# robustrobotics/multi_view_stereonet

Measured on AMD Instinct MI355X. Metric: depthmaps/sec at 512x256, 64 hypotheses, 2 src views; L1 vs ref, higher is better.
Workload: dtype f32; 1 GPU; GTA-SfM-shaped 512x256, D=64 hypotheses, 2 source views, cost-volume filter + 5 refiners; global_batch=256, parallelism=dp1 (independent images, all-gather of metric rows)

## Files before the change

### multi_view_stereonet_amd/csrc/mvsn_conv_wino.hip

```cpp
#include <type_traits>
#include <utility>

#include "mvsn_resident.h"
#include "mvsn_conv_wino.h"

namespace mvsn {

constexpr int WN_THREADS = 512, WN_WAVES = 8;
constexpr int WN_TY = 16, WN_TX = 32;
constexpr int WN_WIDE_TY = 10, WN_WIDE_TX = 40, WN_WIDE_PC = WN_WIDE_TX / 2, WN_WIDE_NP = (WN_WIDE_TY / 2) * WN_WIDE_PC;
constexpr int WN_ROLL_PR = 6, WN_ROLL_NP = WN_ROLL_PR * WN_WIDE_PC, WN_ROLL_HY = 2 * WN_ROLL_PR + 3;
constexpr int WN_TILE_RP = 3;
constexpr int wn_pa(int dil) { return (dil + 3) / 4 * 4; }
constexpr int WN_UFLOATS = 16 * 128;
constexpr int WN_MAX_CHUNKS = 9;
constexpr int WN_LDS_MAX = 160 * 1024;

__device__ floatx4 g_wn_zero16 = {0.f, 0.f, 0.f, 0.f};

#ifndef MVSN_WN_ABLATE
#define MVSN_WN_ABLATE 0
#endif

#ifndef MVSN_RD_ABLATE
// ... 796 lines not shown
#pragma unroll
      for (int rr = 0; rr < 2; ++rr) {
        const bool rok = rr ? row1 : row0;
#pragma unroll
        for (int h = 0; h < 2; ++h) {
          const bool ok = rok && (h ? q1 : q0);
          if (rok && (!(MVSN_WN_ABLATE & 64) || n < 0))
            wn_store4<MVSN_WN_NT_STORES ? 2 : 0>(
                osrd, h ? ovoff1 : ovoff0, (unsigned)(((size_t)(t * 16) * cstride + (size_t)rr * DIL * g.W) * 4),
                floatx4{y[t][rr][4 * h], y[t][rr][4 * h + 1], y[t][rr][4 * h + 2], y[t][rr][4 * h + 3]});
          if (ok) {
#pragma unroll
            for (int k = 0; k < 4; ++k) s[t] += y[t][rr][4 * h + k];
          }
        }
      }
    }
    WN_STAMP();
    if (out_partials != nullptr) {
      auto sum8 = [](float v) {
        v += dpp_mov<0xB1>(v);
        v += dpp_mov<0x4E>(v);
        v += dpp_mov<0x141>(v);
        return v;
      };
      const int hi = (lq >> 3) & 1;
      const float npos = 8.0f * (float)cnt;
      const float rn = cnt == 16 ? 0.0078125f : (cnt == 8 ? 0.015625f : (cnt == 4 ? 0.03125f : 0.0f));
      float m[2], qv[2] = {0.f, 0.f};
#pragma unroll
      for (int t = 0; t < 2; ++t) {
        s[t] = sum8(s[t]);
        m[t] = s[t] * rn;
      }
#pragma unroll
      for (int t = 0; t < 2; ++t)
#pragma unroll
        for (int rr = 0; rr < 2; ++rr)
#pragma unroll
          for (int h = 0; h < 2; ++h)
            if ((rr ? row1 : row0) && (h ? q1 : q0)) {
#pragma unroll
              for (int k = 0; k < 4; ++k) {
                const float dv = y[t][rr][4 * h + k] - m[t];
                qv[t] += dv * dv;
              }
            }
#pragma unroll
      for (int t = 0; t < 2; ++t) qv[t] = sum8(qv[t]);
      int rtile = tile_id, rwave = wave;
      bool rec_ok = true;
      if constexpr (RP) {
        const int yq = oy & (TY - 1);
        rtile = (oy / TY) * g.ntx + x0 / TX, rwave = yq / (2 * DIL) * DIL + yq % DIL;
        rec_ok = oy < g.nty * TY;
      }
      if ((lq & 7) == 0 && rec_ok) {
        float *rec = out_partials + (((size_t)n * (RP ? g.tiles : ptiles) + (size_t)z * g.tiles + rtile) * WN_WAVES + rwave) * 48;
        rec += gq * 12 + hi * 3;
#pragma unroll
        for (int t = 0; t < 2; ++t) {
          rec[t * 6 + 0] = npos;
          rec[t * 6 + 1] = m[t];
          rec[t * 6 + 2] = qv[t];
        }
      }
    }
  };

  auto finish_tile_tr = [&](int n, int z, int tile_id, int y0, int x0, int r_s) {
    int lq;
    asm volatile("v_mbcnt_lo_u32_b32 %0, -1, 0\n\tv_mbcnt_hi_u32_b32 %0, -1, %0" : "=v"(lq));
    const int pc = lq & 15, gq = lq >> 4;
    int oy = y0 + 2 * wave, ox = x0 + 2 * pc;
    bool slot_ok = true;
    unsigned zb = 0;
    if constexpr (WIDE != 0) {
      const int q = wave * 16 + pc;
      slot_ok = q < NP;
      const int qq = slot_ok ? q : 0, pr = qq / WN_WIDE_PC;
      oy = y0 + 2 * pr, ox = x0 + 2 * (qq - pr * WN_WIDE_PC);
      if constexpr (ROLL) {
        const bool pb = pr >= r_s;
        oy = pb ? 2 * (pr - r_s) : oy;
        zb = pb ? (unsigned)plane : 0u;
        slot_ok = slot_ok & (!pb | (z + 1 < g.D));
      }
    }
    const bool row0 = oy < g.H, row1 = oy + 1 < g.H, cok = slot_ok && ox < g.W;
    const size_t cstride = VOL ? (size_t)g.D * plane : plane;
    const __amdgpu_buffer_rsrc_t osrd = wn_rsrc(out + (size_t)n * 32 * cstride + (size_t)z * plane, (unsigned)(32 * cstride * 4));
    const unsigned ovoff = cok ? ((unsigned)(4 * gq) * (unsigned)cstride + zb + (unsigned)(oy * g.W + ox)) * 4u : 0xFFFFFFFFu;
    const unsigned ovoff0 = (!WIDE || row0) ? ovoff : 0xFFFFFFFFu, ovoff1 = (!WIDE || row1) ? ovoff : 0xFFFFFFFFu;
    float s[2] = {0.f, 0.f};
    float y[2][4][4];
#pragma unroll
    for (int t = 0; t < 2; ++t) {
      const floatx4 bv = *reinterpret_cast<const floatx4 *>(bias_lds + t * 16 + 4 * gq);
#pragma unroll
      for (int r = 0; r < 4; ++r) {
        float s0[4], s1[4];
#pragma unroll
        for (int j = 0; j < 4; ++j) {
          s0[j] = acc[j][t][r] + acc[4 + j][t][r] + acc[8 + j][t][r];
          s1[j] = acc[4 + j][t][r] - acc[8 + j][t][r] - acc[12 + j][t][r];
        }
        y[t][r][0] = s0[0] + s0[1] + s0[2] + bv[r];
        y[t][r][1] = s0[1] - s0[2] - s0[3] + bv[r];
        y[t][r][2] = s1[0] + s1[1] + s1[2] + bv[r];
        y[t][r][3] = s1[1] - s1[2] - s1[3] + bv[r];
        if (!(MVSN_WN_ABLATE & 64) || n < 0) {
          const unsigned so = (unsigned)((size_t)(t * 16 + r) * cstride * 4);
          if (WIDE || row0) wn_store2<MVSN_WN_NT_TR ? 2 : 0>(osrd, ovoff0, so, y[t][r][0], y[t][r][1]);
          if (WIDE || row1) wn_store2<MVSN_WN_NT_TR ? 2 : 0>(osrd, ovoff1, so + (unsigned)g.W * 4u, y[t][r][2], y[t][r][3]);
        }
        if (row0 && cok) s[t] += y[t][r][0] + y[t][r][1];
        if (row1 && cok) s[t] += y[t][r][2] + y[t][r][3];
      }
    }
    WN_STAMP();
    if (out_partials != nullptr) {
      auto sum16 = [](float v) {
        v += dpp_mov<0xB1>(v);
        v += dpp_mov<0x4E>(v);
        v += dpp_mov<0x141>(v);
        v += dpp_mov<0x140>(v);
        return v;
      };
      const int vp = (g.W - x0) >> 1;
      float npos = (float)(8 * ((row0 ? 1 : 0) + (row1 ? 1 : 0)) * (vp > 16 ? 16 : vp));
      if constexpr (WIDE != 0)
        npos = sum16(cok ? (float)(8 * ((row0 ? 1 : 0) + (row1 ? 1 : 0))) : 0.0f);
      float m[2], qv[2] = {0.f, 0.f};
#pragma unroll
      for (int t = 0; t < 2; ++t) {
        s[t] = sum16(s[t]);
        m[t] = npos > 0.f ? s[t] / npos : 0.f;
      }
#pragma unroll
      for (int t = 0; t < 2; ++t)
#pragma unroll
        for (int r = 0; r < 4; ++r)
#pragma unroll
          for (int k = 0; k < 4; ++k)
            if ((k < 2 ? row0 : row1) && cok) {
              const float dv = y[t][r][k] - m[t];
              qv[t] += dv * dv;
            }
#pragma unroll
      for (int t = 0; t < 2; ++t) qv[t] = sum16(qv[t]);
      if (pc < 4) {
        float *rec = out_partials + (((size_t)n * ptiles + (ROLL ? (size_t)0 : (size_t)z * g.tiles) + tile_id) * WN_WAVES + wave) * 48;
        rec += gq * 12 + pc * 3;
        const int ga = gq >> 1;
        const bool a = pc == ga, b = pc == 2 + ga;
        rec[0] = (a || b) ? npos : 0.f;
        rec[1] = a ? m[0] : (b ? m[1] : 0.f);
        rec[2] = a ? qv[0] : (b ? qv[1] : 0.f);
      }
    }
  };

  int step = 0, mm_stage = 0;
  for (int round = 0; round < my_items; ++round) {
#ifdef MVSN_WN_STAMPS
    dbg_on = round >= 3 || my_items < 4;
#endif
    const int flat = g.rev ? total - 1 - (round * G + slot) : round * G + slot;
    const int n = flat / ptiles;
    int tile_id = flat - n * ptiles, z = 0;
    int r_pr0 = 0, r_s = WN_ROLL_PR;
    if constexpr (ROLL) {
      roll_item(tile_id, z, r_pr0, r_s);
    } else if constexpr (VOL) {
      z = tile_id / g.tiles;
      tile_id -= z * g.tiles;
    }
    const int tyi = ROLL ? 0 : wdiv(tile_id, g.fd_ntx), txi = ROLL ? 0 : tile_id - tyi * g.ntx;
    const int y0 = ROLL ? 2 * r_pr0 : item_y0(tyi), x0 = txi * TX;

#pragma unroll
    for (int xi = 0; xi < 16; ++xi) asm volatile("" : "=v"(acc[xi][0]), "=v"(acc[xi][1]));

    int chunk = 0;
    auto do_step = [&](auto firstc) {
      const bool has_next = step + 1 < total_steps;
      bool waited = false;
      if constexpr (RIDE > 0) {
        if constexpr (ASM_RIDE) {
          if (rd_young != PERV) asm volatile("s_waitcnt vmcnt(0)" ::: "memory");
          asm volatile("s_waitcnt vmcnt(%0)" ::"n"(PERV) : "memory");
        } else if (rd_young == PERV) asm volatile("s_waitcnt vmcnt(%0)" ::"n"(PERV) : "memory");
        else if (rd_young == PER) asm volatile("s_waitcnt vmcnt(%0)" ::"n"(PER) : "memory");
        else if (VOL && rd_young == 2) asm volatile("s_waitcnt vmcnt(2)" ::: "memory");
        else asm volatile("s_waitcnt vmcnt(0)" ::: "memory");
        rd_consume(lane);
        waited = true;
      }
      if (has_next) {
        const int rest = total_steps - (step + 2);
        if (!waited) wait_landed(rest < 0 ? 0 : (rest < NSTAGE - 2 ? rest : NSTAGE - 2));
        xf_apply();
        WN_STAMP();
        if (!(MVSN_WN_ABLATE & 8)) wn_barrier<LDS_BARRIER>();
        if (MVSN_WN_STAGGER > 0 && wave >= 4) __builtin_amdgcn_s_sleep(MVSN_WN_STAGGER);
        WN_STAMP();
        xf_prepare();
      }
      rd_issue(flat, chunk);
      float dn[KS][4][4];
      if (has_next && !(MVSN_WN_ABLATE & 32)) {
        if (MVSN_WN_XF == 1) tr_load(dn);
        else if (MVSN_WN_XF == 0) tr_load(dn, 0, 1);
      }
      auto multiply = [&](auto first, auto hc) {
        constexpr bool FIRST = decltype(first)::value;
        constexpr int h = decltype(hc)::value;
        const float *ub = U + (VOL ? mm_stage : chunk) * UST + h * WN_UFLOATS + lane;
        float fb[2][2];
        fb[0][0] = ub[0], fb[0][1] = ub[64];
        auto tcol = [&](int i, int j) {
          const float d0 = dn[h][0][dslot(j)], d1 = dn[h][1][dslot(j)], d2 = dn[h][2][dslot(j)], d3 = dn[h][3][dslot(j)];
          return i == 0 ? d0 - d2 : (i == 1 ? d1 + d2 : (i == 2 ? d2 - d1 : d1 - d3));
        };
        constexpr bool INTER = MVSN_WN_XF == 1 || (MVSN_WN_XF == 0 && h == 0);
        float tc[4], tn[4];
        if constexpr (INTER) {
#pragma unroll
          for (int j = 0; j < 4; ++j) tc[j] = tcol(0, j);
        } else {
          if (has_next && !(MVSN_WN_ABLATE & 32)) tr_load(dn, h, h + 1);
        }
#pragma unroll
        for (int xi = 0; xi < 16; ++xi) {
          const int cur = xi & 1, ti = xi >> 2, tj = xi & 3;
          if (INTER && ti < 3) tn[tj] = tcol(ti + 1, tj);
          if (xi + 1 < 16 && !(MVSN_WN_ABLATE & 2)) {
            fb[cur ^ 1][0] = ub[(xi + 1) * 128];
            fb[cur ^ 1][1] = ub[(xi + 1) * 128 + 64];
          }
          if constexpr (FIRST) {
            acc[xi][0] = TR ? mfma16x16x4(fb[cur][0], v[h][xi], floatx4{0.f, 0.f, 0.f, 0.f})
                            : mfma16x16x4(v[h][xi], fb[cur][0], floatx4{0.f, 0.f, 0.f, 0.f});
            acc[xi][1] = TR ? mfma16x16x4(fb[cur][1], v[h][xi], floatx4{0.f, 0.f, 0.f, 0.f})
                            : mfma16x16x4(v[h][xi], fb[cur][1], floatx4{0.f, 0.f, 0.f, 0.f});
          } else {
            acc[xi][0] = TR ? mfma16x16x4(fb[cur][0], v[h][xi], acc[xi][0]) : mfma16x16x4(v[h][xi], fb[cur][0], acc[xi][0]);
            acc[xi][1] = TR ? mfma16x16x4(fb[cur][1], v[h][xi], acc[xi][1]) : mfma16x16x4(v[h][xi], fb[cur][1], acc[xi][1]);
          }
          if (h == 0 && xi == 1 && has_next && !(MVSN_WN_ABLATE & 4)) {
            pf_issue();
            uq_issue();
          }
          if constexpr (INTER) {
            if (!(MVSN_WN_ABLATE & 1)) {
              v[h][xi] = tj == 0 ? tc[0] - tc[2] : (tj == 1 ? tc[1] + tc[2] : (tj == 2 ? tc[2] - tc[1] : tc[1] - tc[3]));
              if (MVSN_WN_PIN) asm volatile("" : "+v"(v[h][xi]));
            }
            if (tj == 3) {
#pragma unroll
              for (int k = 0; k < 4; ++k) tc[k] = tn[k];
            }
          }
          __builtin_amdgcn_sched_barrier(0);
        }
        if constexpr (!INTER) {
          if (!(MVSN_WN_ABLATE & 1)) {
            tr_finish(dn, v, h, h + 1);
#pragma unroll
            for (int xi = 0; xi < 16; ++xi)
              if (MVSN_WN_PIN) asm volatile("" : "+v"(v[h][xi]));
          }
          __builtin_amdgcn_sched_barrier(0);
        }
      };
      multiply(firstc, std::integral_constant<int, 0>{});
      if constexpr (KS == 2) multiply(std::false_type{}, std::integral_constant<int, 1>{});
      tr_advance();
      if constexpr (VOL) mm_stage = mm_stage + 1 == NSTAGE ? 0 : mm_stage + 1;
      WN_STAMP();
      ++step;
    };
    do_step(std::true_type{});
    for (chunk = 1; chunk < nsteps; ++chunk) do_step(std::false_type{});
    if (!(MVSN_WN_ABLATE & 16) || n < 0) {
      if constexpr (TR) finish_tile_tr(n, z, tile_id, y0, x0, r_s);
      else finish_tile(n, z, tile_id, y0, x0);
    }
  }
  if constexpr (RIDE > 0) {
    if (total_steps > 0) {
      asm volatile("s_waitcnt vmcnt(0)" ::: "memory");
      int ln;
      asm volatile("v_mbcnt_lo_u32_b32 %0, -1, 0\n\tv_mbcnt_hi_u32_b32 %0, -1, %0" : "=v"(ln));
      rd_consume(ln);
    }
  }
#ifdef MVSN_WN_STAMPS
  if (dbg)
    for (int i = 0; i < dbg_i; ++i) dbg[i] = dbg_lds[i];
#endif
}

constexpr int S2_TY = 16, S2_TX = 32;
constexpr int S2_ROWS = 2 * S2_TY + 3, S2_XS = 2 * S2_TX + 8, S2_DQ = S2_XS / 4;
constexpr int S2_GROUPS = S2_ROWS * S2_DQ, S2_PIECES = (S2_GROUPS + 63) / 64;
constexpr int S2_RCST = S2_ROWS * S2_XS + 1;
constexpr int S2_STAGE = 4 * S2_RCST;
constexpr int S2_UST = 4 * WN_UFLOATS;
constexpr int S2_STEPS = 8;
constexpr size_t S2_LDS_BYTES = (size_t)(2 * S2_STAGE + 2 * S2_UST + 32) * sizeof(float);
static_assert(S2_PIECES * 4 % WN_WAVES == 0, "a step's raw pieces divide evenly among the waves");
static_assert(S2_LDS_BYTES <= 160 * 1024, "LDS plan");

__global__ void wino_s2_pack_kernel(const float *__restrict__ w, float *__restrict__ out) {
  const int idx = blockIdx.x * blockDim.x + threadIdx.x;
  if (idx >= S2_STEPS * S2_UST) return;
  const int lane = idx & 63, t = (idx >> 6) & 1, xi = (idx >> 7) & 15, ph = (idx >> 11) & 3, cc = idx >> 13;
  const int py = ph >> 1, px = ph & 1;
  const int co = t * 16 + (lane & 15), ci = cc * 4 + (lane >> 4);
  const float *g = w + ((size_t)co * 32 + ci) * 25;
  const float G[4][3] = {{1.f, 0.f, 0.f}, {0.5f, 0.5f, 0.5f}, {0.5f, -0.5f, 0.5f}, {0.f, 0.f, 1.f}};
  const int i = xi >> 2, j = xi & 3;
  float u = 0.0f;
  for (int a = 0; a < 3; ++a)
    for (int b = 0; b < 3; ++b) {
      const int ky = 2 * a + py, kx = 2 * b + px;
      if (ky < 5 && kx < 5) u += G[i][a] * g[ky * 5 + kx] * G[j][b];
    }
  out[idx] = u;
}

#ifndef MVSN_S2_PIN
#define MVSN_S2_PIN 1
#endif
#ifndef MVSN_S2_CNTWAIT
#define MVSN_S2_CNTWAIT 1
#endif
struct WinoS2Args {
  int n, H, W, Ho, Wo, ntx, tiles;
  WinoDiv fd_ntx;
};

__global__ __launch_bounds__(WN_THREADS, 2) void conv_wino_s2_kernel(WinoS2Args g, const float *__restrict__ in,
                                                                     const float *__restrict__ upk,
                                                                     const float *__restrict__ bias,
                                                                     float *__restrict__ out) {
  extern __shared__ __attribute__((aligned(16))) float smem[];
  float *U = smem + 2 * S2_STAGE;
  float *bias_lds = U + 2 * S2_UST;
  const int tid = threadIdx.x, lane = tid & 63;
  const int wave = __builtin_amdgcn_readfirstlane(tid >> 6);
  const size_t plane = (size_t)g.H * g.W;
  const int oplane = g.Ho * g.Wo;
  const int total = g.n * g.tiles, G = gridDim.x;
  const int slot = xcd_tile_index(blockIdx.x, G);
  const int my_items = slot < total ? (total - slot + G - 1) / G : 0;
  const int total_steps = my_items * S2_STEPS;
  if (tid < 32) bias_lds[tid] = bias ? bias[tid] : 0.0f;

  constexpr int PER = S2_PIECES * 4 / WN_WAVES;
  const int dch = wave >> 1, dp0 = (wave & 1) * PER;
  int pf_item = 0, pf_cc = 0, pf_n = 0;
  int pf_goff[PER];
  auto pf_plan = [&]() {
    const int flat = pf_item * G + slot;
    const int n = flat / g.tiles, tile = flat - n * g.tiles;
    const int tyi = wdiv(tile, g.fd_ntx), txi = tile - tyi * g.ntx;
    const int gy0 = 2 * tyi * S2_TY - 2, gx0 = 2 * txi * S2_TX - 4;
    pf_n = n;
    int lo;
    asm volatile("v_mbcnt_lo_u32_b32 %0, -1, 0\n\tv_mbcnt_hi_u32_b32 %0, -1, %0" : "=v"(lo));
#pragma unroll
    for (int i = 0; i < PER; ++i) {
      const int e = (dp0 + i) * 64 + lo;
      const int row = e / S2_DQ, q = e - row * S2_DQ;
      const int gy = gy0 + row, gx = gx0 + 4 * q;
      pf_goff[i] = (gy >= 0 && gy < g.H && gx >= 0 && gx < g.W) ? (gy * g.W + gx) * 4 : -1;
    }
  };
  auto pf_issue = [&](int step) {
    if (step >= total_steps) return;
    const float *src = in + ((size_t)pf_n * 32 + pf_cc * 4 + dch) * plane;
    float *dst = smem + (step & 1) * S2_STAGE + dch * S2_RCST;
#pragma unroll
    for (int i = 0; i < PER; ++i)
      if ((dp0 + i) * 64 + lane < S2_GROUPS)
        wn_dma16_buf<true>(src, (unsigned)plane * 4u, (unsigned)pf_goff[i], dst + (dp0 + i) * 256);
    const float *us = upk + (size_t)pf_cc * S2_UST + wave * 1024 + lane * 4;
    float *ud = U + (step & 1) * S2_UST + wave * 1024;
#pragma unroll
    for (int i = 0; i < 4; ++i) wn_dma16<true>(us + i * 256, ud + i * 256);
    if (++pf_cc == S2_STEPS) {
      pf_cc = 0;
      ++pf_item;
      if (pf_item < my_items) pf_plan();
    }
  };
  if (my_items > 0) pf_plan();
  pf_issue(0);

  const int pcol = lane & 15, kc = lane >> 4;
  const int rbase = kc * S2_RCST + (4 * wave) * S2_XS + 4 * pcol + 2;

  floatx4 acc[16][2];
#pragma unroll
  for (int xi = 0; xi < 16; ++xi) acc[xi][0] = acc[xi][1] = floatx4{0.f, 0.f, 0.f, 0.f};

  int item = 0, cc = 0;
  for (int step = 0; step < total_steps; ++step) {
    if (MVSN_S2_CNTWAIT && cc == 0 && step > 0) asm volatile("s_waitcnt vmcnt(8)" ::: "memory");
    else asm volatile("s_waitcnt vmcnt(0)" ::: "memory");
    wn_barrier<true>();
    pf_issue(step + 1);
    const float *raw = smem + (step & 1) * S2_STAGE + rbase;
    const float *us = U + (step & 1) * S2_UST + lane;
#pragma unroll
    for (int py = 0; py < 2; ++py) {
      typedef float s2_f2 __attribute__((ext_vector_type(2)));
      s2_f2 d[4][4];
#pragma unroll
      for (int i = 0; i < 4; ++i)
#pragma unroll
        for (int j = 0; j < 4; ++j) {
          const float *q = raw + (py + 2 * i) * S2_XS + 2 * j;
          d[i][j] = (py && i == 3) ? s2_f2{0.f, 0.f} : s2_f2{q[0], q[1]};
        }
      s2_f2 t[4][4], v[16];
#pragma unroll
      for (int j = 0; j < 4; ++j) {
        t[0][j] = d[0][j] - d[2][j];
        t[1][j] = d[1][j] + d[2][j];
        t[2][j] = d[2][j] - d[1][j];
        t[3][j] = d[1][j] - d[3][j];
      }
#pragma unroll
      for (int i = 0; i < 4; ++i) {
        v[i * 4 + 0] = t[i][0] - t[i][2];
        v[i * 4 + 1] = t[i][1] + t[i][2];
        v[i * 4 + 2] = t[i][2] - t[i][1];
        v[i * 4 + 3] = t[i][1] - t[i][3];
      }
      if (MVSN_S2_PIN) {
#pragma unroll
        for (int xi = 0; xi < 16; ++xi)
          if (!(py && (xi >> 2) == 3)) asm volatile("" : "+v"(v[xi]));
      }
#pragma unroll
      for (int xi = 0; xi < 16; ++xi) {
        if (py && (xi >> 2) == 3) continue;
        const float *u = us + ((py * 2) * 16 + xi) * 128;
        acc[xi][0] = mfma16x16x4(v[xi].x, u[0], acc[xi][0]);
        acc[xi][1] = mfma16x16x4(v[xi].x, u[64], acc[xi][1]);
        if ((xi & 3) != 3) {
          acc[xi][0] = mfma16x16x4(v[xi].y, u[16 * 128], acc[xi][0]);
          acc[xi][1] = mfma16x16x4(v[xi].y, u[16 * 128 + 64], acc[xi][1]);
        }
      }
    }
    if (++cc == S2_STEPS) {
      cc = 0;
      const int flat = item * G + slot;
      const int n = flat / g.tiles, tile = flat - n * g.tiles;
      const int tyi = wdiv(tile, g.fd_ntx), txi = tile - tyi * g.ntx;
      const int y0 = tyi * S2_TY + 2 * wave, x0 = txi * S2_TX;
      const __amdgpu_buffer_rsrc_t osrd = wn_rsrc(out + (size_t)n * 32 * oplane, (unsigned)(32 * oplane) * 4u);
      int lo;
      asm volatile("v_mbcnt_lo_u32_b32 %0, -1, 0\n\tv_mbcnt_hi_u32_b32 %0, -1, %0" : "=v"(lo));
      const int ocl = lo & 15, oq = lo >> 4;
      unsigned ovoff[2];
#pragma unroll
      for (int hx = 0; hx < 2; ++hx)
        ovoff[hx] = x0 + 8 * oq + 4 * hx < g.Wo ? (unsigned)((ocl * oplane + 8 * oq + 4 * hx) * 4) : 0xFFFFFFFFu;
#pragma unroll
      for (int tt = 0; tt < 2; ++tt) {
        const float bv = bias_lds[tt * 16 + ocl];
        float y[4][2][2];
#pragma unroll
        for (int r = 0; r < 4; ++r) {
          float tm[2][4];
#pragma unroll
          for (int j = 0; j < 4; ++j) {
            tm[0][j] = acc[0 + j][tt][r] + acc[4 + j][tt][r] + acc[8 + j][tt][r];
            tm[1][j] = acc[4 + j][tt][r] - acc[8 + j][tt][r] - acc[12 + j][tt][r];
          }
#pragma unroll
          for (int a = 0; a < 2; ++a) {
            y[r][a][0] = tm[a][0] + tm[a][1] + tm[a][2] + bv;
            y[r][a][1] = tm[a][1] - tm[a][2] - tm[a][3] + bv;
          }
        }
#pragma unroll
        for (int a = 0; a < 2; ++a) {
          const bool rok = y0 + a < g.Ho;
          const unsigned so = rok ? (unsigned)((tt * 16 * oplane + (y0 + a) * g.Wo + x0) * 4) : 0u;
          wn_store4<0>(osrd, rok ? ovoff[0] : 0xFFFFFFFFu, so, floatx4{y[0][a][0], y[0][a][1], y[1][a][0], y[1][a][1]});
          wn_store4<0>(osrd, rok ? ovoff[1] : 0xFFFFFFFFu, so, floatx4{y[2][a][0], y[2][a][1], y[3][a][0], y[3][a][1]});
        }
      }
#pragma unroll
      for (int xi = 0; xi < 16; ++xi) acc[xi][0] = acc[xi][1] = floatx4{0.f, 0.f, 0.f, 0.f};
      ++item;
    }
  }
}

static int g_wn_rowphase = 0;

bool wino_geom(const mvsn_conv_desc *d, WinoGeom *g) {
  if (!d || d->precision != MVSN_CONV_FP32_WINO) return false;
  g->rpy = 0;
  if (d->n <= 0 || d->c_in <= 0 || d->c_out != 32 || d->depth < 1 || d->rows <= 0 || d->cols <= 0) return false;
  g->s2 = false;
  if (d->kd == 1 && d->kh == 5 && d->kw == 5 && d->stride == 2) {
    if (d->c_in != 32 || d->dilation != 1 || d->depth != 1 || d->cols % 8 != 0) return false;
    if ((unsigned long long)d->rows * d->cols * 32ull * 4ull >= (1ull << 31)) return false;
    g->s2 = true, g->wide = 0;
    g->n = d->n, g->cin = 32, g->H = d->rows, g->W = d->cols, g->dil = 1, g->D = 1, g->vol = false;
    g->nty = ((d->rows - 1) / 2 + 1 + S2_TY - 1) / S2_TY;
    g->ntx = ((d->cols - 1) / 2 + 1 + S2_TX - 1) / S2_TX;
    g->tiles = g->nty * g->ntx;
    g->nchunks = S2_STEPS * 4;
    g->packed_floats = (size_t)S2_STEPS * S2_UST;
    return (long)g->n * g->tiles < (1L << 30);
  }
  if ((d->kd != 1 && d->kd != 3) || d->kh != 3 || d->kw != 3 || d->stride != 1) return false;
  if (d->kd == 1 && d->depth != 1) return false;
  if (d->dilation != 1 && d->dilation != 2 && d->dilation != 4 && d->dilation != 8) return false;
  if (d->cols % 4 != 0) return false;
  if ((unsigned long long)d->depth * d->rows * d->cols * 32ull * 4ull >= (1ull << 32)) return false;
  g->n = d->n, g->cin = d->c_in, g->H = d->rows, g->W = d->cols, g->dil = d->dilation;
  g->D = d->depth, g->vol = d->kd == 3;
  g->nty = (d->rows + WN_TY - 1) / WN_TY;
  g->ntx = (d->cols + WN_TX - 1) / WN_TX;
  g->wide = 0;
#ifndef MVSN_WN_NO_WIDE
  if (d->kd == 3 && d->cols > WN_TX && d->cols <= WN_WIDE_TX) {
    const int strips = (d->rows + WN_WIDE_TY - 1) / WN_WIDE_TY;
    if (strips < g->nty * g->ntx) g->wide = 1, g->nty = strips, g->ntx = 1;
  }
#endif
  g->tiles = g->nty * g->ntx;
#ifndef MVSN_WN_NO_ROLL
  if (d->kd == 3 && d->cols > WN_TX && d->cols <= WN_WIDE_TX && d->c_in == 32 && d->dilation == 1) {
    const int pr = (d->rows + 1) / 2;
    const long items = ((long)d->depth * pr + WN_ROLL_PR - 1) / WN_ROLL_PR;
    if (pr >= WN_ROLL_PR && items < (long)d->depth * g->tiles && items < (1L << 24))
      g->wide = 2, g->nty = 1, g->ntx = 1, g->tiles = (int)items;
  }
#endif
  if (g->vol) {
    if (d->c_in != 32 || d->dilation != 1) return false;
    if ((long)wino_items(*g) > 1L << 24) return false;
    g->nchunks = 24;
    g->packed_floats = (size_t)g->nchunks * WN_UFLOATS;
    return true;
  }
  g->nchunks = (d->c_in + 3) / 4;
  if (g->nchunks > WN_MAX_CHUNKS) return false;
  if (g->nchunks > 8 && d->dilation > 2) return false;
  if (g->nchunks == 1 && d->dilation != 1) return false;
  g->packed_floats = (size_t)g->nchunks * WN_UFLOATS;
#ifndef MVSN_WN_NO_ROWPHASE
  if (d->dilation > 1 && g_wn_rowphase != 2) {
    const int rpy = ((d->rows + d->dilation - 1) / d->dilation + WN_TY - 1) / WN_TY;
    if (g_wn_rowphase == 1 || d->dilation * rpy <= g->nty) g->rpy = rpy;
  }
#endif
  return true;
}

int wino_pack_2d(const float *weight, int cin, float *packed, hipStream_t stream) {
  const int nchunks = (cin + 3) / 4, total = nchunks * WN_UFLOATS;
  hipLaunchKernelGGL(wino_pack_kernel, dim3((total + 255) / 256), dim3(256), 0, stream, weight, cin, 32, nchunks, 1,
                     packed);
  return check_launch("wino_pack_2d");
}

int wino_pack(const mvsn_conv_desc *d, const float *weight, float *packed, hipStream_t stream) {
  WinoGeom g;
  if (!wino_geom(d, &g)) return MVSN_E_BADARG;
  if (g.s2) {
    hipLaunchKernelGGL(wino_s2_pack_kernel, dim3((S2_STEPS * S2_UST + 255) / 256), dim3(256), 0, stream, weight, packed);
    return check_launch("mvsn_conv_pack_weights(winograd, 5x5 stride 2)");
  }
  const int total = g.nchunks * WN_UFLOATS;
  hipLaunchKernelGGL(wino_pack_kernel, dim3((total + 255) / 256), dim3(256), 0, stream, weight, g.cin, 32, g.nchunks,
                     g.vol ? 3 : 1, packed);
  return check_launch("mvsn_conv_pack_weights(winograd)");
}

static int wino_select(const WinoGeom &g, bool job) {
  if (g.s2) return -1;
  const bool head = g.nchunks == 1, rp = g.rpy > 0;
  WinoForm f = {};
  f.dil = g.dil, f.vol = g.vol, f.tile = rp ? WN_TILE_RP : g.wide;
  f.fullw = MVSN_WN_FULLW_OK && g.vol && !g.wide && g.ntx == 1 && g.W <= WN_TX;
  f.ks = (head || (rp ? job && g.dil == 8 : g.dil == 8 || (job && g.dil == 4))) ? 1 : 2;
  const bool four = !job && ((!g.vol && g.nchunks <= 8 && (rp ? g.dil <= 4 : g.dil == 1)) || g.wide == 2);
  f.nstage = head ? 6 : (four ? 4 : 3);
  f.ride = !job ? 0 : (g.vol ? 1 : (g.nchunks == 8 ? f.ks : 0));
  if (job && !f.ride) return -1;
  const int row = wn_find_form(f);
  return row >= 0 && g.nchunks <= WN_FORMS[row].chunks ? row : -1;
}

bool wino_can_carry(const WinoGeom &g, const mvsn_apply_job *job) {
  const int row = wino_select(g, true);
  if (row < 0 || !job || !job->x || !job->stats || !job->gamma || !job->beta || !job->out || job->n <= 0) return false;
  const int r = WN_FORMS[row].ride;
  if (job->spatial <= 0 || job->spatial % (256 * r) != 0) return false;
  if (job->r_stats && !(job->residual && job->r_gamma && job->r_beta)) return false;
  if ((((size_t)job->x | (size_t)job->out | (size_t)job->residual) & 15) != 0) return false;
  const long units = (long)job->n * 32 * (job->spatial / 256);
  if (g.vol && job->residual) return false;
  const long capacity = (long)g.n * wino_work_items(g) * WN_FORMS[row].nsteps(g.nchunks) * WN_WAVES * r;
  return units <= capacity && capacity < (1L << 31) && units < (1L << 30);
}

int wino_launch(const WinoGeom &g, const float *in, const float *upk, const float *bias, const float *in_stats,
                const float *in_gamma, const float *in_beta, float *out, float *out_partials, hipStream_t stream,
                const WinoBlocks *blocks, const mvsn_apply_job *job) {
  if (g.s2) {
    if (blocks || job || in_stats || out_partials) {
      set_error("mvsn_conv_forward(winograd, 5x5 stride 2): no input transform, statistics, channel blocks or carried job");
      return MVSN_E_BADARG;
    }
    WinoS2Args a;
    a.n = g.n, a.H = g.H, a.W = g.W, a.Ho = (g.H - 1) / 2 + 1, a.Wo = (g.W - 1) / 2 + 1, a.ntx = g.ntx, a.tiles = g.tiles;
    a.fd_ntx = wino_div((unsigned)g.ntx);
    static LdsOptIn opt;
    if (int rc = ensure_lds(opt, (const void *)conv_wino_s2_kernel, S2_LDS_BYTES, "mvsn_conv_forward(winograd, 5x5 stride 2)"))
      return rc;
    const long total = (long)g.n * g.tiles;
    const int cus = device_cus();
    hipLaunchKernelGGL(conv_wino_s2_kernel, dim3((unsigned)(total < cus ? total : cus)), dim3(WN_THREADS), S2_LDS_BYTES,
                       stream, a, in, upk, bias, out);
    return check_launch("mvsn_conv_forward(winograd, 5x5 stride 2)");
  }
  RideArgs rd = {};
  if (job) {
    if (blocks || !wino_can_carry(g, job)) {
      set_error("mvsn_conv_forward(winograd): this launch cannot carry the job");
      return MVSN_E_BADARG;
    }
    rd.x = job->x, rd.stats = job->stats, rd.gamma = job->gamma, rd.beta = job->beta;
    rd.res = job->residual, rd.r_stats = job->r_stats, rd.r_gamma = job->r_gamma, rd.r_beta = job->r_beta;
    rd.out = job->out;
    rd.units = (int)((long)job->n * 32 * (job->spatial / 256));
    rd.fd_upp = wino_div((unsigned)(job->spatial / 256));
  }
  WinoArgs a;
  a.n = g.n, a.cin = g.cin, a.H = g.H, a.W = g.W, a.ntx = g.ntx, a.tiles = g.tiles, a.nchunks = g.nchunks;
  a.fd_ntx = wino_div((unsigned)g.ntx);
  a.cb0 = g.cin, a.cb1 = 0, a.in1 = a.in2 = in;
  a.D = g.D;
  a.pr = (g.H + 1) / 2, a.fd_pr = wino_div((unsigned)a.pr);
  a.nty = g.nty, a.rpy = g.rpy;
  if (blocks) a.cb0 = blocks->cb0, a.cb1 = blocks->cb1, a.in1 = blocks->in1, a.in2 = blocks->in2;
  a.rev = (job && job->reverse == 1) ? 1 : 0;
  a.cs0 = (size_t)g.H * g.W, a.bs0 = (size_t)a.cb0 * a.cs0;
  if (blocks && blocks->cs0) a.cs0 = blocks->cs0, a.bs0 = blocks->bs0;
  const int row = wino_select(g, job != nullptr);
  if (row < 0) {
    set_error("mvsn_conv_forward(winograd): no kernel form for this layer");
    return MVSN_E_BADARG;
  }
  const size_t lds = WN_FORMS[row].bytes(g.nchunks);
  const int cus = device_cus();
  const long total = (long)g.n * wino_work_items(g);
  const dim3 grid((unsigned)(total < cus ? total : cus));
  auto launch = [&](auto mode, auto I) -> int {
    constexpr WinoForm F = WN_FORMS[decltype(I)::value];
    const auto kernel = conv_wino_kernel<decltype(mode)::value, F.ks, F.nstage, F.dil, F.vol, F.ride, F.tile, F.fullw>;
    static LdsOptIn opt;
    if (int rc = ensure_lds(opt, (const void *)kernel, lds, "mvsn_conv_forward(winograd)")) return rc;
    hipLaunchKernelGGL(kernel, grid, dim3(WN_THREADS), lds, stream, a, in, upk, bias, in_stats, in_gamma, in_beta, out,
                       out_partials, rd, (const void *)a.in1, (const void *)a.in2, (const void *)rd.x,
                       (const void *)rd.stats, (const void *)rd.res, (const void *)rd.r_stats, (const void *)rd.out,
                       (const void *)nullptr, (const void *)nullptr, (const void *)nullptr);
    return 0;
  };
  const bool xf = in_stats != nullptr;
  if (int rc = with_form_row(row, std::make_index_sequence<WN_NFORMS>{}, [&](auto I) {
        return xf ? launch(std::integral_constant<int, 1>{}, I) : launch(std::integral_constant<int, 0>{}, I);
      }))
    return rc;
  return check_launch("mvsn_conv_forward(winograd)");
}

}

extern "C" int mvsn_debug_set_wino_rowphase(int mode) {
  const int old = mvsn::g_wn_rowphase;
  mvsn::g_wn_rowphase = mode;
  return old;
}

extern "C" int mvsn_debug_wino_plan(const mvsn_conv_desc *desc, int carrying, int out[8]) {
  mvsn::WinoGeom g;
  if (!out || !mvsn::wino_geom(desc, &g)) return 0;
  const int row = mvsn::wino_select(g, carrying != 0);
  if (row < 0) return 0;
  const mvsn::WinoForm &f = mvsn::WN_FORMS[row];
  out[0] = f.ks, out[1] = f.nstage, out[2] = f.ride, out[3] = f.tile, out[4] = f.fullw;
  out[5] = (int)f.bytes(g.nchunks), out[6] = (int)mvsn::wino_work_items(g), out[7] = f.nsteps(g.nchunks);
  return 1;
}

#ifdef MVSN_WN_STAMPS
extern "C" int mvsn_debug_set_wino_stamps(void *buf) {
  return (int)hipMemcpyToSymbol(HIP_SYMBOL(mvsn::g_wn_stamps), &buf, sizeof(buf));
}
#endif
```

Before: 3851 depthmaps/s.

## Split stride-2 5x5 Winograd conv by row phase and drop zero coefficient blocks

Makes a row-phase decomposition the default for the 5x5 stride-2 Winograd conv, keeping the old kernel behind a macro. Each channel quad is processed as two half-steps, one per input row phase, with half the raw rows staged. The weight blocks that are identically zero for odd phases are removed (49 of 64 kept), which cuts MFMA count and weight traffic. It also adds a three-deep LDS ring and overlaps the next input transform with the current MFMAs, at the cost of more LDS, more registers and more complex wait and barrier logic.

```diff
diff --git a/multi_view_stereonet_amd/csrc/mvsn_conv_wino.hip b/multi_view_stereonet_amd/csrc/mvsn_conv_wino.hip
--- a/multi_view_stereonet_amd/csrc/mvsn_conv_wino.hip
+++ b/multi_view_stereonet_amd/csrc/mvsn_conv_wino.hip
@@ -1122,6 +1122,19 @@
 #endif
 }
 
+#ifndef MVSN_S2_PIN
+#define MVSN_S2_PIN 1
+#endif
+#ifndef MVSN_S2_CNTWAIT
+#define MVSN_S2_CNTWAIT 1
+#endif
+struct WinoS2Args {
+  int n, H, W, Ho, Wo, ntx, tiles;
+  WinoDiv fd_ntx;
+};
+constexpr int S2_QUADS = 8;
+
+#ifdef MVSN_S2_NO_ROWPHASE
 constexpr int S2_TY = 16, S2_TX = 32;
 constexpr int S2_ROWS = 2 * S2_TY + 3, S2_XS = 2 * S2_TX + 8, S2_DQ = S2_XS / 4;
 constexpr int S2_GROUPS = S2_ROWS * S2_DQ, S2_PIECES = (S2_GROUPS + 63) / 64;
@@ -1150,17 +1163,6 @@
     }
   out[idx] = u;
 }
-
-#ifndef MVSN_S2_PIN
-#define MVSN_S2_PIN 1
-#endif
-#ifndef MVSN_S2_CNTWAIT
-#define MVSN_S2_CNTWAIT 1
-#endif
-struct WinoS2Args {
-  int n, H, W, Ho, Wo, ntx, tiles;
-  WinoDiv fd_ntx;
-};
 
 __global__ __launch_bounds__(WN_THREADS, 2) void conv_wino_s2_kernel(WinoS2Args g, const float *__restrict__ in,
                                                                      const float *__restrict__ upk,
@@ -1324,6 +1326,269 @@
     }
   }
 }
+constexpr int S2_PACKED_FLOATS = S2_STEPS * S2_UST;
+
+#else
+
+#ifndef MVSN_S2_STAGES
+#define MVSN_S2_STAGES 3
+#endif
+#ifndef MVSN_S2_XF
+#define MVSN_S2_XF 1
+#endif
+constexpr int S2_TY = 16, S2_TX = 32;
+constexpr int S2_XS = 2 * S2_TX + 8, S2_DQ = S2_XS / 4;
+constexpr int S2_PROWS = S2_TY + 2;
+constexpr int s2_groups(int py) { return (S2_PROWS - py) * S2_DQ; }
+constexpr int S2_PIECES = (s2_groups(0) + 63) / 64;
+constexpr int S2_RCST = S2_PROWS * S2_XS + 1;
+constexpr int S2_STAGE = 4 * S2_RCST;
+constexpr bool s2_kept(int py, int xi, int px) { return !(py && (xi >> 2) == 3) && !(px && (xi & 3) == 3); }
+constexpr int s2_blk(int py, int xi, int px) {
+  int n = 0;
+  for (int x = 0; x < 16; ++x)
+    for (int p = 0; p < 2; ++p) {
+      if (x == xi && p == px) return n;
+      n += s2_kept(py, x, p);
+    }
+  return n;
+}
+constexpr int S2_UBLK0 = s2_blk(0, 16, 0), S2_UBLK1 = s2_blk(1, 16, 0);
+constexpr int S2_UST = S2_UBLK0 * 128;
+constexpr int S2_UCC = (S2_UBLK0 + S2_UBLK1) * 128;
+constexpr int S2_STEPS = 2 * S2_QUADS;
+constexpr int S2_PACKED_FLOATS = S2_QUADS * S2_UCC;
+constexpr int S2_NST = MVSN_S2_STAGES;
+constexpr size_t S2_LDS_BYTES = (size_t)(S2_NST * S2_STAGE + S2_NST * S2_UST + 32) * sizeof(float);
+static_assert(S2_UBLK0 == 28 && S2_UBLK1 == 21, "49 of the 64 coefficient blocks of a channel quad remain");
+static_assert(S2_NST == 2 || S2_NST == 3, "ring depth");
+static_assert(S2_STAGE % 4 == 0 && S2_UBLK0 * 32 % 4 == 0 && S2_UBLK1 * 32 % 4 == 0, "16-byte DMA slots");
+static_assert(S2_LDS_BYTES <= 160 * 1024, "LDS plan");
+
+__global__ void wino_s2_pack_kernel(const float *__restrict__ w, float *__restrict__ out) {
+  const int idx = blockIdx.x * blockDim.x + threadIdx.x;
+  if (idx >= S2_PACKED_FLOATS) return;
+  const int cc = idx / S2_UCC, r = idx - cc * S2_UCC;
+  const int py = r >= S2_UST, blk = (r - py * S2_UST) >> 7;
+  const int lane = r & 63, t = (r >> 6) & 1;
+  int xi = 0, px = 0, nb = 0;
+  for (int x = 0; x < 16; ++x)
+    for (int p = 0; p < 2; ++p)
+      if (s2_kept(py, x, p)) {
+        if (nb == blk) xi = x, px = p;
+        ++nb;
+      }
+  const int co = t * 16 + (lane & 15), ci = cc * 4 + (lane >> 4);
+  const float *g = w + ((size_t)co * 32 + ci) * 25;
+  const float G[4][3] = {{1.f, 0.f, 0.f}, {0.5f, 0.5f, 0.5f}, {0.5f, -0.5f, 0.5f}, {0.f, 0.f, 1.f}};
+  const int i = xi >> 2, j = xi & 3;
+  float u = 0.0f;
+  for (int a = 0; a < 3; ++a)
+    for (int b = 0; b < 3; ++b) {
+      const int ky = 2 * a + py, kx = 2 * b + px;
+      if (ky < 5 && kx < 5) u += G[i][a] * g[ky * 5 + kx] * G[j][b];
+    }
+  out[idx] = u;
+}
+
+__global__ __launch_bounds__(WN_THREADS, 2) void conv_wino_s2_kernel(WinoS2Args g, const float *__restrict__ in,
+                                                                     const float *__restrict__ upk,
+                                                                     const float *__restrict__ bias,
+                                                                     float *__restrict__ out) {
+  constexpr int NST = S2_NST, XF = MVSN_S2_XF ? 1 : 0, RA = NST - 1 + XF, UA = NST - 1;
+  extern __shared__ __attribute__((aligned(16))) float smem[];
+  float *U = smem + NST * S2_STAGE;
+  float *bias_lds = U + NST * S2_UST;
+  const int tid = threadIdx.x, lane = tid & 63;
+  const int wave = __builtin_amdgcn_readfirstlane(tid >> 6);
+  const size_t plane = (size_t)g.H * g.W;
+  const int oplane = g.Ho * g.Wo;
+  const int total = g.n * g.tiles, G = gridDim.x;
+  const int slot = xcd_tile_index(blockIdx.x, G);
+  const int my_items = slot < total ? (total - slot + G - 1) / G : 0;
+  const int total_steps = my_items * S2_STEPS;
+  if (tid < 32) bias_lds[tid] = bias ? bias[tid] : 0.0f;
+
+  const int fg = wave >> 2, dch = wave & 3;
+  const int fgroups = fg ? s2_groups(1) : s2_groups(0);
+  const int upy = fg ^ XF;
+  const int ush = (upy ? S2_UBLK1 : S2_UBLK0) * 32;
+  int pf_item = 0, pf_cc = 0, pf_n = 0, pf_ucc = 0;
+  int pf_goff[S2_PIECES];
+  auto pf_plan = [&]() {
+    const int flat = pf_item * G + slot;
+    const int n = flat / g.tiles, tile = flat - n * g.tiles;
+    const int tyi = wdiv(tile, g.fd_ntx), txi = tile - tyi * g.ntx;
+    const int gy0 = 2 * tyi * S2_TY - 2 + fg, gx0 = 2 * txi * S2_TX - 4;
+    pf_n = n;
+    int lo;
+    asm volatile("v_mbcnt_lo_u32_b32 %0, -1, 0\n\tv_mbcnt_hi_u32_b32 %0, -1, %0" : "=v"(lo));
+#pragma unroll
+    for (int i = 0; i < S2_PIECES; ++i) {
+      const int e = i * 64 + lo;
+      const int row = e / S2_DQ, q = e - row * S2_DQ;
+      const int gy = gy0 + 2 * row, gx = gx0 + 4 * q;
+      pf_goff[i] = (gy >= 0 && gy < g.H && gx >= 0 && gx < g.W) ? (gy * g.W + gx) * 4 : -1;
+    }
+  };
+  auto issue_raw = [&](int s, int stage) {
+    if ((s & 1) != fg || s >= total_steps) return;
+    const float *src = in + ((size_t)pf_n * 32 + pf_cc * 4 + dch) * plane;
+    float *dst = smem + stage * S2_STAGE + dch * S2_RCST;
+#pragma unroll
+    for (int i = 0; i < S2_PIECES; ++i)
+      if (i * 64 + 63 < s2_groups(1) || i * 64 + lane < fgroups)
+        wn_dma16_buf<true>(src, (unsigned)plane * 4u, (unsigned)pf_goff[i], dst + i * 256);
+    if (++pf_cc == S2_QUADS) {
+      pf_cc = 0;
+      ++pf_item;
+      if (pf_item < my_items) pf_plan();
+    }
+  };
+  auto issue_u = [&](int s, int stage) {
+    if (((s & 1) ^ XF) != fg || s >= total_steps) return;
+    const float *us = upk + (size_t)pf_ucc * S2_UCC + upy * S2_UST + dch * ush + lane * 4;
+    float *ud = U + stage * S2_UST + dch * ush;
+#pragma unroll
+    for (int i = 0; i < 4; ++i)
+      if (i * 256 + 252 < S2_UBLK1 * 32 || i * 256 + lane * 4 < ush) wn_dma16<true>(us + i * 256, ud + i * 256);
+    if (++pf_ucc == S2_QUADS) pf_ucc = 0;
+  };
+  if (my_items > 0) pf_plan();
+#pragma unroll
+  for (int s = 0; s < RA; ++s) issue_raw(s, s % NST);
+#pragma unroll
+  for (int s = 0; s < UA; ++s) issue_u(s, s);
+
+  const int pcol = lane & 15, kc = lane >> 4;
+  const int rbase = kc * S2_RCST + (2 * wave) * S2_XS + 4 * pcol + 2;
+
+  typedef float s2_f2 __attribute__((ext_vector_type(2)));
+  s2_f2 v[16];
+  auto transform = [&](auto pyc, int stage) {
+    constexpr int py = decltype(pyc)::value;
+    const float *raw = smem + stage * S2_STAGE + rbase;
+    s2_f2 d[4][4];
+#pragma unroll
+    for (int i = 0; i < 4; ++i)
+#pragma unroll
+      for (int j = 0; j < 4; ++j) {
+        const float *q = raw + i * S2_XS + 2 * j;
+        d[i][j] = (py && i == 3) ? s2_f2{0.f, 0.f} : s2_f2{q[0], q[1]};
+      }
+    s2_f2 t[4][4];
+#pragma unroll
+    for (int j = 0; j < 4; ++j) {
+      t[0][j] = d[0][j] - d[2][j];
+      t[1][j] = d[1][j] + d[2][j];
+      t[2][j] = d[2][j] - d[1][j];
+      t[3][j] = d[1][j] - d[3][j];
+    }
+#pragma unroll
+    for (int i = 0; i < 4; ++i) {
+      v[i * 4 + 0] = t[i][0] - t[i][2];
+      v[i * 4 + 1] = t[i][1] + t[i][2];
+      v[i * 4 + 2] = t[i][2] - t[i][1];
+      v[i * 4 + 3] = t[i][1] - t[i][3];
+    }
+    if (MVSN_S2_PIN) {
+#pragma unroll
+      for (int xi = 0; xi < 16; ++xi)
+        if (!(py && (xi >> 2) == 3)) asm volatile("" : "+v"(v[xi]));
+    }
+  };
+
+  floatx4 acc[16][2];
+#pragma unroll
+  for (int xi = 0; xi < 16; ++xi) acc[xi][0] = acc[xi][1] = floatx4{0.f, 0.f, 0.f, 0.f};
+
+  if (XF) {
+    asm volatile("s_waitcnt vmcnt(0)" ::: "memory");
+    wn_barrier<true>();
+    if (total_steps > 0) transform(std::integral_constant<int, 0>{}, 0);
+  }
+
+  int item = 0, cc = 0, st = 0;
+  auto half = [&](auto pyc, int step) {
+    constexpr int py = decltype(pyc)::value;
+    if (fg == (py ^ XF)) {
+      if (py == 0 && MVSN_S2_CNTWAIT && cc == 0 && step > 0) asm volatile("s_waitcnt vmcnt(8)" ::: "memory");
+      else asm volatile("s_waitcnt vmcnt(0)" ::: "memory");
+    }
+    wn_barrier<true>();
+    const int prev = st == 0 ? NST - 1 : st - 1, next = st + 1 == NST ? 0 : st + 1;
+    issue_raw(step + RA, XF ? st : prev);
+    issue_u(step + UA, prev);
+    if (!XF) transform(pyc, st);
+    const float *us = U + st * S2_UST + lane;
+#pragma unroll
+    for (int xi = 0; xi < 16; ++xi) {
+      if (py && (xi >> 2) == 3) continue;
+      const float *u = us + s2_blk(py, xi, 0) * 128;
+      acc[xi][0] = mfma16x16x4(v[xi].x, u[0], acc[xi][0]);
+      acc[xi][1] = mfma16x16x4(v[xi].x, u[64], acc[xi][1]);
+      if ((xi & 3) != 3) {
+        acc[xi][0] = mfma16x16x4(v[xi].y, u[128], acc[xi][0]);
+        acc[xi][1] = mfma16x16x4(v[xi].y, u[128 + 64], acc[xi][1]);
+      }
+    }
+    if (XF) {
+      __builtin_amdgcn_sched_barrier(0);
+      if (py == 0 || step + 1 < total_steps) transform(std::integral_constant<int, 1 - py>{}, next);
+      __builtin_amdgcn_sched_barrier(0);
+    }
+    st = next;
+  };
+  for (int step = 0; step < total_steps; step += 2) {
+    half(std::integral_constant<int, 0>{}, step);
+    half(std::integral_constant<int, 1>{}, step + 1);
+    if (++cc == S2_QUADS) {
+      cc = 0;
+      const int flat = item * G + slot;
+      const int n = flat / g.tiles, tile = flat - n * g.tiles;
+      const int tyi = wdiv(tile, g.fd_ntx), txi = tile - tyi * g.ntx;
+      const int y0 = tyi * S2_TY + 2 * wave, x0 = txi * S2_TX;
+      const __amdgpu_buffer_rsrc_t osrd = wn_rsrc(out + (size_t)n * 32 * oplane, (unsigned)(32 * oplane) * 4u);
+      int lo;
+      asm volatile("v_mbcnt_lo_u32_b32 %0, -1, 0\n\tv_mbcnt_hi_u32_b32 %0, -1, %0" : "=v"(lo));
+      const int ocl = lo & 15, oq = lo >> 4;
+      unsigned ovoff[2];
+#pragma unroll
+      for (int hx = 0; hx < 2; ++hx)
+        ovoff[hx] = x0 + 8 * oq + 4 * hx < g.Wo ? (unsigned)((ocl * oplane + 8 * oq + 4 * hx) * 4) : 0xFFFFFFFFu;
+#pragma unroll
+      for (int tt = 0; tt < 2; ++tt) {
+        const float bv = bias_lds[tt * 16 + ocl];
+        float y[4][2][2];
+#pragma unroll
+        for (int r = 0; r < 4; ++r) {
+          float tm[2][4];
+#pragma unroll
+          for (int j = 0; j < 4; ++j) {
+            tm[0][j] = acc[0 + j][tt][r] + acc[4 + j][tt][r] + acc[8 + j][tt][r];
+            tm[1][j] = acc[4 + j][tt][r] - acc[8 + j][tt][r] - acc[12 + j][tt][r];
+          }
+#pragma unroll
+          for (int a = 0; a < 2; ++a) {
+            y[r][a][0] = tm[a][0] + tm[a][1] + tm[a][2] + bv;
+            y[r][a][1] = tm[a][1] - tm[a][2] - tm[a][3] + bv;
+          }
+        }
+#pragma unroll
+        for (int a = 0; a < 2; ++a) {
+          const bool rok = y0 + a < g.Ho;
+          const unsigned so = rok ? (unsigned)((tt * 16 * oplane + (y0 + a) * g.Wo + x0) * 4) : 0u;
+          wn_store4<0>(osrd, rok ? ovoff[0] : 0xFFFFFFFFu, so, floatx4{y[0][a][0], y[0][a][1], y[1][a][0], y[1][a][1]});
+          wn_store4<0>(osrd, rok ? ovoff[1] : 0xFFFFFFFFu, so, floatx4{y[2][a][0], y[2][a][1], y[3][a][0], y[3][a][1]});
+        }
+      }
+#pragma unroll
+      for (int xi = 0; xi < 16; ++xi) acc[xi][0] = acc[xi][1] = floatx4{0.f, 0.f, 0.f, 0.f};
+      ++item;
+    }
+  }
+}
+#endif
 
 static int g_wn_rowphase = 0;
 
@@ -1340,8 +1605,8 @@
     g->nty = ((d->rows - 1) / 2 + 1 + S2_TY - 1) / S2_TY;
     g->ntx = ((d->cols - 1) / 2 + 1 + S2_TX - 1) / S2_TX;
     g->tiles = g->nty * g->ntx;
-    g->nchunks = S2_STEPS * 4;
-    g->packed_floats = (size_t)S2_STEPS * S2_UST;
+    g->nchunks = S2_QUADS * 4;
+    g->packed_floats = (size_t)S2_PACKED_FLOATS;
     return (long)g->n * g->tiles < (1L << 30);
   }
   if ((d->kd != 1 && d->kd != 3) || d->kh != 3 || d->kw != 3 || d->stride != 1) return false;
@@ -1401,7 +1666,7 @@
   WinoGeom g;
   if (!wino_geom(d, &g)) return MVSN_E_BADARG;
   if (g.s2) {
-    hipLaunchKernelGGL(wino_s2_pack_kernel, dim3((S2_STEPS * S2_UST + 255) / 256), dim3(256), 0, stream, weight, packed);
+    hipLaunchKernelGGL(wino_s2_pack_kernel, dim3((S2_PACKED_FLOATS + 255) / 256), dim3(256), 0, stream, weight, packed);
     return check_launch("mvsn_conv_pack_weights(winograd, 5x5 stride 2)");
   }
   const int total = g.nchunks * WN_UFLOATS;
```

After: 3852 depthmaps/s, median of 2. About the same (+0.0%).
